# abmoRobotics/isaac_rover_orbit

Hardware: AMD Instinct MI355X
Metric: env-steps/sec AAURoverEnv-v0 @ num_envs=4096; 1/2/4/8 MI355X (higher is better)
Workload: dtype f32

## Files before the change

### isaac_rover_orbit_amd/csrc/rover_kernels.hip

```cpp
#include <hip/hip_runtime.h>
#include <vector>

#include <cmath>
#include <cstdio>
#include <cstring>
#include <new>
#include <type_traits>

#include <dlfcn.h>

#include "../../include/rover_hip.h"
#include "../../include/rover_debug.h"
#include "rover_model.hpp"
#include "rover_internal.hpp"

namespace {

struct StepConsts {
    float h, inv_h, inv_m, inv_I[3];
    float steer_hkp, steer_den_inv, steer_i_over_h, steer_dv_max;
    float wheel_den_inv, wheel_h_over_i, lt_motor;
    float bogie_keep[3], b_winv[3];
    float bogie_gq[3];
};
// ... 402 lines not shown

struct ArmConsts {
    float d0[3], axd[3], ad;
};
__device__ __forceinline__ ArmConsts make_arm(const float *wb, const float *P, const float *ax)
{
    ArmConsts a;
#pragma unroll
    for (int i = 0; i < 3; ++i) a.d0[i] = wb[i] - P[i];
    cross3f(ax, a.d0, a.axd);
    a.ad = dot3f(ax, a.d0);
    return a;
}
struct SubConsts {
    float e1[3], e2[3];
};
__device__ __forceinline__ SubConsts make_sub(const float *cj, const float *P, const float *ax)
{
    const ArmConsts a = make_arm(cj, P, ax);
    SubConsts s;
#pragma unroll
    for (int i = 0; i < 3; ++i) { s.e1[i] = fmaf(ax[i], a.ad, -a.d0[i]); s.e2[i] = a.axd[i]; }
    return s;
}
__device__ __forceinline__ float bogie_gravity(const SubConsts &sub, const float R[3][3], float sb, float cb, float gq, float bd)
{
    float vb[3];
#pragma unroll
    for (int i = 0; i < 3; ++i) vb[i] = fmaf(sub.e1[i], sb, sub.e2[i] * cb);
    const float vwz = fmaf(R[2][2], vb[2], fmaf(R[2][1], vb[1], R[2][0] * vb[0]));
    return fmaf(gq, vwz, bd);
}
__device__ __forceinline__ void bogie_sincos(float bq, float *sb, float *cb)
{
    rv_sincosf_small(bq, sb, cb);
    const bool wide = !(fabsf(bq) < 0.75f);
    if (__builtin_expect(__builtin_amdgcn_ballot_w64(wide) != 0ull, 0)) {
        float s2, c2;
        rv_sincosf(bq, &s2, &c2);
        if (wide) { *sb = s2; *cb = c2; }
    }
}
struct RowQ {
    float ja[3], jb, m;
};
__device__ __forceinline__ RowQ row_quantities(const StepConsts &k, const float R[3][3], const float *r, const float *axrp,
                                               const float *dir, bool friction_row, bool at_hi, bool at_lo, float b_winv)
{
    RowQ o;
    float x[3];
    cross3f(r, dir, x);
    mat_tvecf(R, x, o.ja);
    float jb = dot3f(dir, axrp);
    const bool lock = friction_row ? (at_hi || at_lo) : ((at_hi && jb > 0.0f) || (at_lo && jb < 0.0f));
    if (lock) jb = 0.0f;
    o.jb = jb;
    o.m = 1.0f / (RV_SPLIT_C * k.inv_m + RV_SPLIT_C * wdot3(o.ja, k.inv_I) + RV_SPLIT_B * (jb * jb * b_winv));
    return o;
}
__device__ __forceinline__ float row_coupling(const StepConsts &k, const RowQ &a, const RowQ &b, float b_winv)
{
    return RV_SPLIT_C * wdot3x(a.ja, b.ja, k.inv_I) + RV_SPLIT_B * (a.jb * b.jb * b_winv);
}
__device__ __forceinline__ float dpp_ror8(float x);
struct LinkSample {
    float h00, h01, h10, h11, o00, o01, o10, o11, fx, fy, z;
};
__device__ __forceinline__ LinkSample link_point_fetch(const RvParams &p, const float R[3][3], const float *pos, const float *P,
                                                       const float *ax, float bq, const float *p0, const float *bogie_sc = nullptr)
{
    float sb, cb;
    if (bogie_sc) { sb = bogie_sc[0]; cb = bogie_sc[1]; }
    else bogie_sincos(bq, &sb, &cb);
    const float d0[3] = {p0[0] - P[0], p0[1] - P[1], p0[2] - P[2]};
    float axd[3], pt_b[3], tmp[3];
    cross3f(ax, d0, axd);
    const float ad = dot3f(ax, d0);
#pragma unroll
    for (int i = 0; i < 3; ++i) pt_b[i] = P[i] + fmaf(ax[i], ad * (1.0f - cb), fmaf(axd[i], sb, d0[i] * cb));
    mat_vecf(R, pt_b, tmp);
    float u = ((pos[0] + tmp[0]) - p.min_x) * p.inv_res;
    float v = ((pos[1] + tmp[1]) - p.min_y) * p.inv_res;
    u = clamp_med3(u, 0.0f, (float)(p.W - 1));
    v = clamp_med3(v, 0.0f, (float)(p.H - 1));
    int j0 = (int)u, i0 = (int)v;
    if (j0 > p.W - 2) j0 = p.W - 2;
    if (i0 > p.H - 2) i0 = p.H - 2;
    const size_t base = (size_t)i0 * p.W + j0;
    const float *q = p.height + base, *o = p.obstacle + base;
    LinkSample s;
    s.fx = u - (float)j0; s.fy = v - (float)i0; s.z = pos[2] + tmp[2];
    s.h00 = q[0]; s.h01 = q[1]; s.h10 = q[p.W]; s.h11 = q[p.W + 1];
    s.o00 = o[0]; s.o01 = o[1]; s.o10 = o[p.W]; s.o11 = o[p.W + 1];
    return s;
}
__device__ __forceinline__ void link_point_eval(const LinkSample &s, float inv_res, float *force)
{
    const float dx0 = s.h01 - s.h00, dx1 = s.h11 - s.h10, dy0 = s.h10 - s.h00, dy1 = s.h11 - s.h01;
    const float hx0 = s.h00 + s.fx * dx0, hx1 = s.h10 + s.fx * dx1;
    const float hgt = hx0 + s.fy * (hx1 - hx0);
    const float gx = (dx0 + s.fy * (dx1 - dx0)) * inv_res;
    const float gy = (dy0 + s.fx * (dy1 - dy0)) * inv_res;
    const float o0 = s.o00 + s.fx * (s.o01 - s.o00), o1 = s.o10 + s.fx * (s.o11 - s.o10);
    const float obst = o0 + s.fy * (o1 - o0);
    const float pen = hgt - s.z;
    const float fk = (obst > RV_OBSTACLE_EPS && pen > 0.0f) ? RV_LINK_STIFFNESS * pen : 0.0f;
    const float fz = fk * rv_rsqrtf(fmaf(gx, gx, fmaf(gy, gy, 1.0f)));
    force[0] = -gx * fz;
    force[1] = -gy * fz;
    force[2] = fz;
}
__device__ __forceinline__ float link_sample_obstacle(const LinkSample &s)
{
    const float o0 = s.o00 + s.fx * (s.o01 - s.o00), o1 = s.o10 + s.fx * (s.o11 - s.o10);
    return o0 + s.fy * (o1 - o0);
}
__device__ __forceinline__ void link_point_force(const RvParams &p, const float R[3][3], const float *pos, const float *P,
                                                 const float *ax, float bq, const float *p0, float *force)
{
    link_point_eval(link_point_fetch(p, R, pos, P, ax, bq, p0), p.inv_res, force);
}
__device__ __forceinline__ void link_body_forces(const float lf[6][2], float *Fb )
{
    Fb[0] = (lf[0][1] + lf[1][0]) + lf[1][1];
    Fb[1] = (lf[2][1] + lf[3][0]) + lf[3][1];
    Fb[2] = lf[4][1] + lf[5][1];
    Fb[3] = lf[0][0]; Fb[4] = lf[2][0]; Fb[5] = lf[4][0]; Fb[6] = lf[5][0];
}
template <bool WANT_OBST, bool GROUP_ROLE = false>
__device__ __forceinline__ void wheel_geometry(const RvParams &p, const StepConsts &k, const float R[3][3], const float *pos,
                                               const float *com_w, const ArmConsts &arm, const float *P, const float *ax,
                                               float b_winv, float bq, bool at_hi, bool at_lo, bool steerable, float steer_q,
                                               Contact &ct, bool role_b = false, const float *bogie_sc = nullptr)
{
    const float *d0 = arm.d0, *axd = arm.axd;
    const float ad = arm.ad;
    float sb, cb;
    if (bogie_sc) { sb = bogie_sc[0]; cb = bogie_sc[1]; }
    else bogie_sincos(bq, &sb, &cb);
    float cen_b[3], cen_w[3], piv_w[3], ax_w[3], tmp[3];
#pragma unroll
    for (int i = 0; i < 3; ++i) cen_b[i] = P[i] + fmaf(ax[i], ad * (1.0f - cb), fmaf(axd[i], sb, d0[i] * cb));
    mat_vecf(R, cen_b, tmp);
#pragma unroll
    for (int i = 0; i < 3; ++i) cen_w[i] = pos[i] + tmp[i];
    mat_vecf(R, P, tmp);
#pragma unroll
    for (int i = 0; i < 3; ++i) piv_w[i] = pos[i] + tmp[i];
    mat_vecf(R, ax, ax_w);
    float hgt, gx, gy;
    ct.obst = 0.0f;
    terrain_sample<WANT_OBST>(p, cen_w[0], cen_w[1], hgt, gx, gy, ct.obst);
    const float inv = rv_rsqrtf(fmaf(gx, gx, fmaf(gy, gy, 1.0f)));
    ct.n[0] = -gx * inv; ct.n[1] = -gy * inv; ct.n[2] = inv;
    const float gap = fmaf(cen_w[2] - hgt, ct.n[2], -RV_WHEEL_CONTACT_RADIUS);
    float cp[3];
#pragma unroll
    for (int i = 0; i < 3; ++i) cp[i] = fmaf(-RV_WHEEL_CONTACT_RADIUS, ct.n[i], cen_w[i]);
    float fwd_b[3] = {1.0f, 0.0f, 0.0f}, fwd[3];
    if (steerable) rv_sincosf(steer_q, &fwd_b[1], &fwd_b[0]);
    mat_vecf(R, fwd_b, fwd);
    const float fn = dot3f(fwd, ct.n);
#pragma unroll
    for (int i = 0; i < 3; ++i) ct.t[i] = fmaf(-fn, ct.n[i], fwd[i]);
    const float tl = dot3f(ct.t, ct.t);
    const float tinv = rv_rsqrtf(fmaxf(tl, 1.0e-12f));
#pragma unroll
    for (int i = 0; i < 3; ++i) ct.t[i] *= tinv;
    cross3f(ct.n, ct.t, ct.s);
    float r[3], rp[3], x[3];
#pragma unroll
    for (int i = 0; i < 3; ++i) { r[i] = cp[i] - com_w[i]; rp[i] = cp[i] - piv_w[i]; }
    cross3f(ax_w, rp, x);
    {
        const float sep = -gap * k.inv_h;
        const float push = RV_BAUMGARTE * (-gap) * k.inv_h;
        ct.bias = gap > 0.0f ? sep : fminf(push, RV_MAX_DEPENETRATION_VEL);
    }
    if (!GROUP_ROLE) {
        const RowQ qn = row_quantities(k, R, r, x, ct.n, false, at_hi, at_lo, b_winv);
        const RowQ qt = row_quantities(k, R, r, x, ct.t, true, at_hi, at_lo, b_winv);
        const RowQ qs = row_quantities(k, R, r, x, ct.s, true, at_hi, at_lo, b_winv);
#pragma unroll
        for (int i = 0; i < 3; ++i) { ct.jn_a[i] = qn.ja[i]; ct.jt_a[i] = qt.ja[i]; ct.js_a[i] = qs.ja[i]; }
        ct.jn_b = qn.jb; ct.jt_b = qt.jb; ct.js_b = qs.jb;
        ct.mn = qn.m; ct.mt = qt.m; ct.ms = qs.m;
        ct.a_nt = row_coupling(k, qn, qt, b_winv);
        ct.a_ns = row_coupling(k, qn, qs, b_winv);
        ct.a_ts = row_coupling(k, qt, qs, b_winv);
    } else {
        const float dx[3] = {role_b ? ct.t[0] : ct.n[0], role_b ? ct.t[1] : ct.n[1], role_b ? ct.t[2] : ct.n[2]};
        const RowQ qx = row_quantities(k, R, r, x, dx, role_b, at_hi, at_lo, b_winv);
        const RowQ qs = row_quantities(k, R, r, x, ct.s, true, at_hi, at_lo, b_winv);
        const float a_xs = row_coupling(k, qx, qs, b_winv);
        RowQ qy;
#pragma unroll
        for (int i = 0; i < 3; ++i) qy.ja[i] = dpp_ror8(qx.ja[i]);
        qy.jb = dpp_ror8(qx.jb);
        qy.m = dpp_ror8(qx.m);
        const float a_ys = dpp_ror8(a_xs);
#pragma unroll
        for (int i = 0; i < 3; ++i) { ct.jn_a[i] = role_b ? qy.ja[i] : qx.ja[i]; ct.jt_a[i] = role_b ? qx.ja[i] : qy.ja[i]; ct.js_a[i] = qs.ja[i]; }
        ct.jn_b = role_b ? qy.jb : qx.jb; ct.jt_b = role_b ? qx.jb : qy.jb; ct.js_b = qs.jb;
        ct.mn = role_b ? qy.m : qx.m; ct.mt = role_b ? qx.m : qy.m; ct.ms = qs.m;
        ct.a_nt = row_coupling(k, qx, qy, b_winv);
        ct.a_ns = role_b ? a_ys : a_xs;
        ct.a_ts = role_b ? a_xs : a_ys;
    }
}

typedef float f2 __attribute__((ext_vector_type(2)));
__device__ __forceinline__ f2 fma2(f2 a, f2 b, f2 c) { return __builtin_elementwise_fma(a, b, c); }
struct RoleRows {
    f2 Jn[2];
    f2 Jts[4];
    f2 Cn, Cts;
    f2 Mn[2], Mt[2], Ms[2];
};
__device__ __forceinline__ void role_partials(const RoleRows &r, const f2 *V, float &pn, float &pt, float &ps)
{
    const f2 p = fma2(r.Jn[1], V[1], fma2(r.Jn[0], V[0], r.Cn));
    pn = p.x + p.y;
    f2 ts = fma2(r.Jts[0], (f2){V[0].x, V[0].x}, r.Cts);
    ts = fma2(r.Jts[1], (f2){V[0].y, V[0].y}, ts);
    ts = fma2(r.Jts[2], (f2){V[1].x, V[1].x}, ts);
    ts = fma2(r.Jts[3], (f2){V[1].y, V[1].y}, ts);
    pt = ts.x;
    ps = ts.y;
}
__device__ __forceinline__ void role_outputs(const RoleRows &r, float dn, float dt, float ds, f2 *o)
// ... 368 lines not shown
    "v_add_f32_dpp v252, v252, v252 row_half_mirror" RV_DPP_FULL                                                       \
    "v_add_f32_dpp v253, v253, v253 row_half_mirror" RV_DPP_FULL                                                       \
    "v_add_f32_dpp v254, v254, v254 row_half_mirror" RV_DPP_LANES_A                                                    \
    "v_add_f32_dpp v255, v255, v255 row_half_mirror" RV_DPP_LANES_A                                                    \
    "v_pk_add_f32 %[v0], %[v0], v[252:253]\n\t"                                                                      \
    "v_pk_add_f32 %[v1], %[v1], v[254:255]\n\t"

#define RV_SOLVER_ASM(TRIPS, BODY)                                                                                                \
    asm volatile(                                                                                                                 \
        ".p2align 5\n\t"                                                                                                        \
        "1:\n\t" BODY "s_cbranch_scc1 1b\n\t"                                                                                  \
        : [v0] "+v"(v0), [v1] "+v"(v1), [ln] "+v"(ln), [lt] "+v"(lt), [ls] "+v"(ls), [cnt] "+s"(TRIPS)                            \
        : [jn0] "v"(rr.Jn[0]), [jn1] "v"(rr.Jn[1]), [jts0] "v"(rr.Jts[0]), [jts1] "v"(rr.Jts[1]), [jts2] "v"(rr.Jts[2]),          \
          [jts3] "v"(rr.Jts[3]), [cn] "v"(rr.Cn), [cts] "v"(rr.Cts), [mn0] "v"(rr.Mn[0]), [mn1] "v"(rr.Mn[1]), [mt0] "v"(rr.Mt[0]), \
          [mt1] "v"(rr.Mt[1]), [ms0] "v"(rr.Ms[0]), [ms1] "v"(rr.Ms[1]), [mn] "v"(ct.mn), [mt] "v"(ct.mt), [ms] "v"(ct.ms),        \
          [ant] "v"(ct.a_nt), [ans] "v"(ct.a_ns), [ats] "v"(ct.a_ts), [mu] "s"(mu), [ltm] "s"(K.lt_motor)                         \
        : "v238", "v239", "v240", "v241", "v242", "v243", "v244", "v245", "v246", "v247", "v248", "v249", "v250", "v251",         \
          "v252", "v253", "v254", "v255", "scc")
#define RV_HALF_A(FILLER) RV_SOLVER_HALF("%[ln]", "v249", "%[lt]", "v251", "%[ls]", "v238", FILLER)
#define RV_HALF_B(FILLER) RV_SOLVER_HALF("v249", "%[ln]", "v251", "%[lt]", "v238", "%[ls]", FILLER)
#ifndef RV_SOLVER_UNROLL
#define RV_SOLVER_UNROLL 8
#endif
__device__ __forceinline__ void solver_iterations_group(const StepConsts &K, Contact &ct, const RoleRows &rr, f2 *V, float mu,
                                                        int iterations)
{
    f2 v0 = V[0], v1 = V[1];
    float ln = ct.ln, lt = ct.lt, ls = ct.ls;
    int rest = iterations;
    if (RV_SOLVER_UNROLL == 8) {
        int octs = rest >> 3;
        rest &= 7;
        if (octs > 0)
            RV_SOLVER_ASM(octs, RV_HALF_A("s_sub_u32 %[cnt], %[cnt], 1\n\t") RV_HALF_B("s_nop 0\n\t") RV_HALF_A("s_nop 0\n\t") RV_HALF_B("s_nop 0\n\t")
                                    RV_HALF_A("s_nop 0\n\t") RV_HALF_B("s_nop 0\n\t") RV_HALF_A("s_nop 0\n\t") RV_HALF_B("s_cmp_lg_u32 %[cnt], 0\n\t"));
    }
    if (RV_SOLVER_UNROLL >= 4) {
        int quads = rest >> 2;
        rest &= 3;
        if (quads > 0)
            RV_SOLVER_ASM(quads, RV_HALF_A("s_sub_u32 %[cnt], %[cnt], 1\n\t") RV_HALF_B("s_nop 0\n\t") RV_HALF_A("s_nop 0\n\t")
                                     RV_HALF_B("s_cmp_lg_u32 %[cnt], 0\n\t"));
    }
    int pairs = rest >> 1;
    if (pairs > 0) RV_SOLVER_ASM(pairs, RV_HALF_A("s_sub_u32 %[cnt], %[cnt], 1\n\t") RV_HALF_B("s_cmp_lg_u32 %[cnt], 0\n\t"));
    V[0] = v0;
    V[1] = v1;
    ct.ln = ln;
    ct.lt = lt;
    ct.ls = ls;
    if (iterations & 1) solver_iteration_generic(K, ct, rr, V, mu);
}

template <bool RECORD_FORCE, bool LINK_ELSEWHERE = false>
__device__ __forceinline__ void physics_substep_group(const RvParams &p, const StepConsts &K, GroupLane &g,
                                                      float *Fw ,
                                                      int sidx = 0)
{
    K1_STAMP(2 + 3 * sidx);
    constexpr float COM_B[3] = RV_COM_B_INIT;
    const float h = K.h;
    const float mu = p.cfg.friction_mu;
    if (g.steerable) steer_joint(K, g.steer_t, g.sq, g.sqd);
    float R[3][3], com_w[3];
#pragma unroll
    for (int i = 0; i < 3; ++i) {
        com_w[i] = g.pos[i] + g.com_off[i];
#pragma unroll
        for (int j = 0; j < 3; ++j) R[i][j] = g.R[i][j];
    }
    float v[3] = {g.linvel[0], g.linvel[1], fmaf(-RV_GRAVITY, h, g.linvel[2])};
    float w[3];
    mat_tvecf(R, g.angvel, w);
    const float bq = g.bq;
    float bd = g.bqd * g.bogie_keep;
    float bsc[2];
    bogie_sincos(bq, &bsc[0], &bsc[1]);
    bd = bogie_gravity(g.sub, R, bsc[0], bsc[1], g.bogie_gq, bd);
    const bool at_hi = bq >= RV_BOGIE_QLIM - 1.0e-5f, at_lo = bq <= -RV_BOGIE_QLIM + 1.0e-5f;
    Contact ct;
    LinkSample ls;
    if (RECORD_FORCE && !LINK_ELSEWHERE) ls = link_point_fetch(p, R, g.pos, g.P, g.ax, bq, g.lp, bsc);
    wheel_geometry<RECORD_FORCE && !LINK_ELSEWHERE, true>(p, K, R, g.pos, com_w, g.arm, g.P, g.ax, g.b_winv, bq, at_hi, at_lo, g.steerable, g.sq, ct, g.role_b, bsc);
    if (RECORD_FORCE && !LINK_ELSEWHERE) link_point_eval(ls, p.inv_res, Fw + 3);
    K1_STAMP(3 + 3 * sidx);
    ct.ln = RV_WARM_START * g.lam;
    ct.lt = 0.0f;
    ct.ls = 0.0f;
    const bool rb = g.role_b;
    RoleRows rr;
    {
        const float cw = RV_WHEEL_CONTACT_RADIUS * g.wqd;
        make_role(ct, rb, g.minv0, g.minv1, cw, rr);
    }
    f2 V[2];
    V[0] = rb ? (f2){v[2], w[2]} : (f2){v[0], w[0]};
    V[1] = rb ? (f2){bd, 0.0f} : (f2){v[1], w[1]};
    {
        const f2 l2 = {ct.ln, ct.ln};
        const f2 o0 = rr.Mn[0] * l2, o1 = rr.Mn[1] * l2;
        float a0 = o0.x, a1 = o0.y, a2 = o1.x, a3 = o1.y;
        slot_sum4(a0, a1, a2, a3);
        V[0] += (f2){a0, a1};
        V[1] += (f2){a2, a3};
    }
    solver_iterations_group(K, ct, rr, V, mu, p.cfg.solver_iterations);
    {
        const float p0x = dpp_ror8(V[0].x), p0y = dpp_ror8(V[0].y), p1x = dpp_ror8(V[1].x), p1y = dpp_ror8(V[1].y);
        v[0] = rb ? p0x : V[0].x; w[0] = rb ? p0y : V[0].y;
        v[1] = rb ? p1x : V[1].x; w[1] = rb ? p1y : V[1].y;
        v[2] = rb ? V[0].x : p0x; w[2] = rb ? V[0].y : p0y;
        bd = rb ? V[1].x : p1x;
    }
    K1_STAMP(4 + 3 * sidx);
    wheel_motor(K, g.wheel_t, ct.lt, g.wq, g.wqd);
    g.lam = ct.ln;
    if (RECORD_FORCE) {
        const bool on = LINK_ELSEWHERE ? true : ct.obst > RV_OBSTACLE_EPS;
#pragma unroll
        for (int i = 0; i < 3; ++i) Fw[i] = on ? fmaf(ct.s[i], ct.ls, fmaf(ct.t[i], ct.lt, ct.n[i] * ct.ln)) * K.inv_h : 0.0f;
    }
    chassis_integrate(h, R, v, w, com_w, g.pos, g.quat, g.linvel, g.angvel, g.R, g.com_off);
    bogie_integrate(h, bq, bd, g.bq, g.bqd);
}

struct ResetDraws {
    int32_t spawn_row;
    float yaw_u;
    const float *theta_u;
    float heading_u;
};

__device__ __forceinline__ void sample_target(const RvParams &p, float ox, float oy, uint32_t gid, uint32_t count, const float *inj_theta,
                                              float &tx_out, float &ty_out, float &tz_out)
{
    const rover_config &c = p.cfg;
// ... 778 lines not shown

template <bool TRI>
__device__ __forceinline__ void scan_single_tile_wave(const RvParams &p, int16_t *tile, int lane, int n_env, int e_base,
                                                      const PrivateWindows &w, float *__restrict__ out, int row_stride, int col0,
                                                      const float2 *__restrict__ ray_xy)
{
    if (n_env <= 0) return;
    private_issue(p, w, 0, tile, lane);
    f2 oxy[PRIVATE_ROUNDS];
#pragma unroll
    for (int m = 0; m < PRIVATE_ROUNDS; ++m) {
        const float2 v = ray_xy[m * 64 + lane];
        oxy[m] = (f2){v.x, v.y};
    }
#pragma unroll
    for (int j = 0; j < 4; ++j) {
        if (j < n_env) {
            asm volatile("s_waitcnt vmcnt(0)" ::: "memory");
            __builtin_amdgcn_wave_barrier();
            private_cast<TRI>(p, w, j, tile, lane, e_base, out, row_stride, col0, oxy, ray_xy);
            if (j + 1 < n_env) {
                asm volatile("s_waitcnt lgkmcnt(0)" ::: "memory");
                private_issue(p, w, j + 1, tile, lane);
            }
        }
    }
}

__device__ __forceinline__ void windows_to_lds(float *win, const ScanWindow &sw, int lane)
{
    if ((lane & 15) == 0) {
        float4 *d = reinterpret_cast<float4 *>(win + (lane >> 4) * 8);
        d[0] = make_float4(sw.px, sw.py, sw.pz, sw.cy);
        d[1] = make_float4(sw.sy, __int_as_float(sw.i_lo), __int_as_float(sw.j_lo), __int_as_float(sw.th | (sw.interior << 15) | (sw.tw4 << 16)));
    }
}
__device__ __forceinline__ void windows_from_lds(const float *win, PrivateWindows &w)
{
#pragma unroll
    for (int j = 0; j < 4; ++j) {
        const float4 d0 = reinterpret_cast<const float4 *>(win + j * 8)[0], d1 = reinterpret_cast<const float4 *>(win + j * 8)[1];
        auto uni = [](float v) { return __int_as_float(__builtin_amdgcn_readfirstlane(__float_as_int(v))); };
        w.px[j] = uni(d0.x); w.py[j] = uni(d0.y); w.pz[j] = uni(d0.z); w.cy[j] = uni(d0.w); w.sy[j] = uni(d1.x);
        w.i_lo[j] = __builtin_amdgcn_readfirstlane(__float_as_int(d1.y)); w.j_lo[j] = __builtin_amdgcn_readfirstlane(__float_as_int(d1.z));
        w.pk[j] = __builtin_amdgcn_readfirstlane(__float_as_int(d1.w));
    }
}
constexpr int RV_HAND = 448;
__device__ __forceinline__ float *fused_win(float *lds, const RvParams &p, int wv)
{
    return reinterpret_cast<float *>(reinterpret_cast<int16_t *>(lds) + (size_t)8 * p.tile_dim * p.tile_pitch) + wv * 64;
}
__device__ __forceinline__ float *fused_link(float *lds, const RvParams &p, int wv) { return fused_win(lds, p, 0) + 256 + wv * RV_HAND; }
template <bool TRI>
__device__ __forceinline__ void scan_copy_wave(const RvParams &p, const float *__restrict__ state, float *lds, int partner, int lane,
                                               float *__restrict__ obs, const float2 *__restrict__ ray_xy)
{
    const int tile_cells = p.tile_dim * p.tile_pitch;
    int16_t *tile0 = reinterpret_cast<int16_t *>(lds) + (size_t)(2 * partner) * tile_cells, *tile1 = tile0 + tile_cells;
    const float *win = fused_win(lds, p, partner);
    const int e_base = (int)(blockIdx.x * 4 + partner) * 4;
    const int n_env = max(0, min(4, p.n - e_base));
    PrivateWindows w;
    f2 oxy[PRIVATE_ROUNDS];
#pragma unroll
    for (int m = 0; m < PRIVATE_ROUNDS; ++m) {
        const float2 v = ray_xy[m * 64 + lane];
        oxy[m] = (f2){v.x, v.y};
    }
    {
        const int e = min(e_base + (lane >> 4), p.n - 1);
        const uint32_t count = __float_as_uint(state[(size_t)ROVER_RESET_COUNT * p.n + e]);
        ResetOutcome ro;
        reset_draw(p, (uint32_t)(p.env_id_offset + e), count, nullptr, ro);
        if ((lane & 15) == 0) {
            float4 *d = reinterpret_cast<float4 *>(fused_link(lds, p, partner) + 256 + (lane >> 4) * 12);
            d[0] = make_float4(ro.px, ro.py, ro.pz, ro.qw);
            d[1] = make_float4(ro.qz, ro.tx, ro.ty, ro.tz);
            d[2] = make_float4(ro.heading_cmd, 0.0f, 0.0f, 0.0f);
        }
    }
    {
        __syncthreads();
        const float *lk = fused_link(lds, p, partner);
        const SlotConst sc = d_SLOT[lane & 7];
        const bool role_b = (lane & 8) != 0;
        const float *pe = lk + (lane >> 4) * 12;
        const float R[3][3] = {{pe[0], pe[1], pe[2]}, {pe[3], pe[4], pe[5]}, {pe[6], pe[7], pe[8]}};
        const float pos[3] = {pe[9], pe[10], pe[11]};
        const float P[3] = {sc.P[0], sc.P[1], sc.P[2]}, ax[3] = {sc.ax[0], sc.ax[1], sc.ax[2]};
        float lp[3];
#pragma unroll
        for (int i = 0; i < 3; ++i) lp[i] = role_b ? sc.lp[1][i] : sc.lp[0][i];
        const float bq = lk[64 + lane];
        float bsc[2];
        bogie_sincos(bq, &bsc[0], &bsc[1]);
        const LinkSample ls = link_point_fetch(p, R, pos, P, ax, bq, lp, bsc);
        const float wbp[3] = {sc.wb[0], sc.wb[1], sc.wb[2]};
        const LinkSample ws = link_point_fetch(p, R, pos, P, ax, bq, wbp, bsc);
        float f3[3];
        link_point_eval(ls, p.inv_res, f3);
        const_cast<float *>(lk)[320 + lane] = f3[0];
        const_cast<float *>(lk)[384 + lane] = f3[1];
        const_cast<float *>(lk)[128 + lane] = f3[2];
        const_cast<float *>(lk)[192 + lane] = link_sample_obstacle(ws);
    }
    K1_LITE(0);
    __syncthreads();
    K1_LITE(1);
    {
// ... 32 lines not shown
        if ((lane & 15) == 0)
            *(volatile __attribute__((address_space(3))) float *)(__attribute__((address_space(3))) float *)(lk + 48 + (lane >> 4) * 4 + 3) = 3.0f;
    }
    K1_LITE(3);
    asm volatile("s_waitcnt vmcnt(0)" ::: "memory");
    K1_LITE(4);
    if (n_env > 0) private_cast<TRI>(p, w, 0, tile0, lane, e_base, obs, p.obs_w, 4, oxy, ray_xy);
    K1_LITE(5);
    asm volatile("s_waitcnt lgkmcnt(0)" ::: "memory");
    K1_LITE(6);
    K1_LITE(7);
    if (n_env > 2) private_issue(p, w, 2, tile0, lane);
    K1_LITE(8);
    asm volatile("s_waitcnt vmcnt(0)" ::: "memory");
    K1_LITE(9);
    K1_LITE(10);
    K1_LITE(11);
    if (n_env > 2) private_cast<TRI>(p, w, 2, tile0, lane, e_base, obs, p.obs_w, 4, oxy, ray_xy);
    K1_LITE(12);
    K1_LITE(13);
    K1_LITE(14);
    K1_LITE(15);
}

enum StepForm { TWO_LAUNCH, COPY_WAVES, SINGLE_TILE };
template <StepForm FORM, bool TRI, bool BEGIN_ONLY = false>
__device__ __forceinline__ void step_group_body(const RvParams &p, float *__restrict__ state, const float *__restrict__ action,
                                                float *__restrict__ obs, float *__restrict__ reward, uint8_t *__restrict__ terminated,
                                                uint8_t *__restrict__ truncated, float *__restrict__ force,
                                                float *__restrict__ log_partial, float *lds, const float2 *__restrict__ ray_xy)
{
    const int lane = threadIdx.x & 63;
    const int wave = blockIdx.x * (RV_K1G_THREADS / 64) + (threadIdx.x >> 6);
    const int e_raw = wave * 4 + (lane >> 4);
    const bool active = e_raw < p.n;
    const int e = active ? e_raw : p.n - 1;
    const int N = p.n;
    const rover_config &c = p.cfg;
    const SlotConst sc = d_SLOT[lane & 7];
    const GroupIds id = group_ids(lane, sc);
    K1_STAMP(0);
    K1_LITE(0);

    const StepConsts &K = p.K;
    GroupLane g;
    group_load(state, N, e, id, sc, K, g, p.cfg.mass_model);
    float act[2], prev[2];
    prev[0] = state[(size_t)(ROVER_ACTION + 0) * N + e];
    prev[1] = state[(size_t)(ROVER_ACTION + 1) * N + e];
    const float2 a = reinterpret_cast<const float2 *>(action)[e];
    act[0] = a.x;
    act[1] = a.y;
    float S[ROVER_STATE_WORDS];
    {
        float processed[2], steer[4], rim[6];
        ackermann_core(c, act, processed, steer, rim);
        const float steer_m[4] = {steer[0], steer[3], steer[1], steer[2]};
        const float rim_m[6] = {rim[1], rim[5], rim[0], rim[4], rim[2], rim[3]};
        float st = steer_m[0], rv = rim_m[0];
#pragma unroll
        for (int i = 1; i < 4; ++i) st = (id.si == i) ? steer_m[i] : st;
#pragma unroll
        for (int i = 1; i < 6; ++i) rv = (id.k == i) ? rim_m[i] : rv;
        g.steer_t = st;
        g.wheel_t = rv / c.wheel_radius;
    }
    float Fw[6] = {0.0f, 0.0f, 0.0f, 0.0f, 0.0f, 0.0f};
    f2 oxy[PRIVATE_ROUNDS];
    K1_STAMP(1);
    for (int s = 0; s < c.decimation - 1; ++s) physics_substep_group<false>(p, K, g, nullptr, s);
#pragma unroll
    for (int i = ROVER_TARGET_W; i < ROVER_ACTION; ++i) S[i] = state[(size_t)i * N + e];
#pragma unroll
    for (int i = ROVER_TIME_LEFT; i < ROVER_LAMBDA_N; ++i) S[i] = state[(size_t)i * N + e];
    S[ROVER_RESET_COUNT] = state[(size_t)ROVER_RESET_COUNT * N + e];
    if constexpr (FORM == COPY_WAVES) {
        const int wv = __builtin_amdgcn_readfirstlane((int)(threadIdx.x >> 6));
        float *lk = fused_link(lds, p, wv);
        if ((lane & 15) == 0) {
            float4 *d = reinterpret_cast<float4 *>(lk + (lane >> 4) * 12);
            d[0] = make_float4(g.R[0][0], g.R[0][1], g.R[0][2], g.R[1][0]);
            d[1] = make_float4(g.R[1][1], g.R[1][2], g.R[2][0], g.R[2][1]);
            d[2] = make_float4(g.R[2][2], g.pos[0], g.pos[1], g.pos[2]);
        }
        lk[64 + lane] = g.bq;
        __syncthreads();
        if (c.decimation > 0) physics_substep_group<true, true>(p, K, g, Fw, c.decimation - 1);
    } else {
        if (c.decimation > 0) physics_substep_group<true>(p, K, g, Fw, c.decimation - 1);
    }
    K1_STAMP(20);
    K1_LITE(1);
    if constexpr (FORM == COPY_WAVES) {
        const int wv = __builtin_amdgcn_readfirstlane((int)(threadIdx.x >> 6));
        float *lk = fused_link(lds, p, wv);
        if ((lane & 15) == 0) {
            float4 *d = reinterpret_cast<float4 *>(lk + 48 + (lane >> 4) * 4);
            float4 *q = reinterpret_cast<float4 *>(lk + 304 + (lane >> 4) * 4);
            d[0] = make_float4(g.pos[0], g.pos[1], g.pos[2], 0.0f);
            q[0] = make_float4(g.quat[0], g.quat[1], g.quat[2], g.quat[3]);
        }
        __syncthreads();
        if (c.decimation > 0) {
            const int wv = __builtin_amdgcn_readfirstlane((int)(threadIdx.x >> 6));
            const float *lk = fused_link(lds, p, wv);
            Fw[3] = lk[320 + lane]; Fw[4] = lk[384 + lane]; Fw[5] = lk[128 + lane];
            if (!(lk[192 + lane] > RV_OBSTACLE_EPS)) { Fw[0] = 0.0f; Fw[1] = 0.0f; Fw[2] = 0.0f; }
        }
    }
    if (!id.wheel_active) { Fw[0] = 0.0f; Fw[1] = 0.0f; Fw[2] = 0.0f; Fw[3] = 0.0f; Fw[4] = 0.0f; Fw[5] = 0.0f; }
    float F[ROVER_NUM_BODIES * 3];
#pragma unroll
    for (int i = 0; i < ROVER_NUM_BODIES * 3; ++i) F[i] = 0.0f;
    const bool any_force = __ballot(Fw[0] != 0.0f || Fw[1] != 0.0f || Fw[2] != 0.0f || Fw[5] != 0.0f) != 0ull;
    if (__builtin_expect(any_force, 0)) {
        constexpr int BODY_SLOT[6] = {1, 3, 0, 2, 4, 5};
        const int base = lane & ~15;
#pragma unroll
        for (int b = 0; b < 6; ++b)
#pragma unroll
            for (int i = 0; i < 3; ++i) F[(7 + b) * 3 + i] = __shfl(Fw[i], base + BODY_SLOT[b], 64);
#pragma unroll
        for (int i = 0; i < 3; ++i) {
            float lf[6][2], Fb[7];
#pragma unroll
            for (int sl = 0; sl < 6; ++sl) {
                lf[sl][0] = __shfl(Fw[3 + i], base + sl, 64);
                lf[sl][1] = __shfl(Fw[3 + i], base + 8 + sl, 64);
            }
            link_body_forces(lf, Fb);
#pragma unroll
            for (int b = 0; b < 7; ++b) F[b * 3 + i] = Fb[b];
        }
    }
    int coll_known = -1;
    if constexpr (FORM == COPY_WAVES) {
        const int wv = __builtin_amdgcn_readfirstlane((int)(threadIdx.x >> 6));
        const bool coll = any_force ? collision_measure(F) > 1.0f : false;
        coll_known = coll ? 1 : 0;
        bool term_e[ROVER_NUM_TERM];
// ... 178 lines not shown
                __builtin_amdgcn_s_sleep(1);
            }
        }
        windows_from_lds(win, pw);
        K1_LITE(5);
        K1_STAMP(27);
        if (n_scan > 1) {
            private_issue(p, pw, 1, tile1, lane);
            asm volatile("s_waitcnt vmcnt(0)" ::: "memory");
            private_cast<TRI>(p, pw, 1, tile1, lane, e_base, obs, p.obs_w, 4, oxy, ray_xy);
            asm volatile("s_waitcnt lgkmcnt(0)" ::: "memory");
        }
        K1_STAMP(28);
        K1_LITE(6);
        K1_LITE(7);
        if (n_scan > 3) {
            private_issue(p, pw, 3, tile1, lane);
            K1_LITE(8);
            asm volatile("s_waitcnt vmcnt(0)" ::: "memory");
            K1_STAMP(29);
            K1_LITE(9);
            private_cast<TRI>(p, pw, 3, tile1, lane, e_base, obs, p.obs_w, 4, oxy, ray_xy);
        }
        K1_STAMP(26);
        K1_LITE(10);
    }
}
__global__ __launch_bounds__(RV_K1G_THREADS) void rover_step_begin_kernel(RvParams p, float *__restrict__ state,
                                                                          const float *__restrict__ action, float *__restrict__ reward,
                                                                          uint8_t *__restrict__ terminated, uint8_t *__restrict__ truncated,
                                                                          float *__restrict__ force)
{
    step_group_body<TWO_LAUNCH, false, true>(p, state, action, nullptr, reward, terminated, truncated, force, nullptr, nullptr, nullptr);
}
__global__ __launch_bounds__(RV_K1G_THREADS) void rover_step_kernel_group(RvParams p, float *__restrict__ state,
                                                              const float *__restrict__ action, float *__restrict__ obs,
                                                              float *__restrict__ reward, uint8_t *__restrict__ terminated,
                                                              uint8_t *__restrict__ truncated, float *__restrict__ force,
                                                              float *__restrict__ log_partial)
{
    step_group_body<TWO_LAUNCH, false>(p, state, action, obs, reward, terminated, truncated, force, log_partial, nullptr, nullptr);
}
template <bool TRI>
__global__ __launch_bounds__(2 * RV_K1G_THREADS) RV_FUSED_ATTR void rover_step_scan_kernel(
    RvParams p, float *__restrict__ state, const float *__restrict__ action, float *__restrict__ obs, float *__restrict__ reward,
    uint8_t *__restrict__ terminated, uint8_t *__restrict__ truncated, float *__restrict__ force, float *__restrict__ log_partial,
    const float2 *__restrict__ ray_xy)
{
    extern __shared__ __align__(16) float lds[];
    const int wv = __builtin_amdgcn_readfirstlane((int)(threadIdx.x >> 6));
    if (wv < RV_K1G_THREADS / 64) {
        step_group_body<COPY_WAVES, TRI>(p, state, action, obs, reward, terminated, truncated, force, log_partial, lds, ray_xy);
    } else {
        scan_copy_wave<TRI>(p, state, lds, wv - RV_K1G_THREADS / 64, (int)(threadIdx.x & 63), obs, ray_xy);
    }
}

__global__ __launch_bounds__(RV_K1G_THREADS) void rover_physics_kernel_group(RvParams p, float *__restrict__ state,
                                                                             const float *steer_t, const float *wheel_t,
                                                                             int substeps, float *force)
{
    const int lane = threadIdx.x & 63;
    const int e_raw = (blockIdx.x * (RV_K1G_THREADS / 64) + (threadIdx.x >> 6)) * 4 + (lane >> 4);
    const bool active = e_raw < p.n;
    const int e = active ? e_raw : p.n - 1;
    const int N = p.n;
    const SlotConst sc = d_SLOT[lane & 7];
    const GroupIds id = group_ids(lane, sc);
    const StepConsts &K = p.K;
    GroupLane g;
    group_load(state, N, e, id, sc, K, g, p.cfg.mass_model);
    g.steer_t = steer_t[4 * e + (id.si >= 0 ? id.si : 0)];
    g.wheel_t = wheel_t[6 * e + id.k];
    float Fw[6] = {0.0f, 0.0f, 0.0f, 0.0f, 0.0f, 0.0f};
    for (int s = 0; s < substeps - 1; ++s) physics_substep_group<false>(p, K, g, nullptr);
    if (substeps > 0) physics_substep_group<true>(p, K, g, Fw);
    if (!id.wheel_active) { Fw[3] = 0.0f; Fw[4] = 0.0f; Fw[5] = 0.0f; }
    if (active) group_store(state, N, e, id, g, lane);
    if (force && active && id.owner) {
#pragma unroll
        for (int i = 0; i < 3; ++i) force[(size_t)(id.body * 3 + i) * N + e] = Fw[i];
    }
    if (force) {
        const int base = lane & ~15;
#pragma unroll
        for (int i = 0; i < 3; ++i) {
            float lf[6][2], Fb[7];
#pragma unroll
            for (int sl = 0; sl < 6; ++sl) {
                lf[sl][0] = __shfl(Fw[3 + i], base + sl, 64);
                lf[sl][1] = __shfl(Fw[3 + i], base + 8 + sl, 64);
            }
            link_body_forces(lf, Fb);
            if (active && (lane & 15) < 7) {
                float fb = Fb[0];
#pragma unroll
                for (int b = 1; b < 7; ++b) fb = ((lane & 15) == b) ? Fb[b] : fb;
                force[(size_t)((lane & 15) * 3 + i) * N + e] = fb;
            }
        }
    }
}

__global__ __launch_bounds__(64) void rover_reset_kernel(RvParams p, float *__restrict__ state, const uint8_t *mask,
                                                         const int32_t *spawn_row, const float *yaw_u, const float *theta_u,
                                                         const float *heading_u)
{
// ... 1252 lines not shown
```

Baseline: 103.5 million.

## Offload steering joint integration and sincos to copy waves via LDS handoff

In the fused scan kernel, the copy waves now precompute the steering-joint integration and steering sin/cos for every substep. They write the results into spare LDS tile rows and publish them through an LDS flag word. The physics waves spin-wait on that flag after the first substep, then read the precomputed steering values instead of recomputing them, which takes that work off the physics critical path. It adds a __syncthreads in the copy path, a spin loop with sleep, and reuse of tile LDS that must not overlap the scan's use of it. There are also small branch-to-select rewrites in row_quantities and in the bias computation.

```diff
diff --git a/isaac_rover_orbit_amd/csrc/rover_kernels.hip b/isaac_rover_orbit_amd/csrc/rover_kernels.hip
--- a/isaac_rover_orbit_amd/csrc/rover_kernels.hip
+++ b/isaac_rover_orbit_amd/csrc/rover_kernels.hip
@@ -478,8 +478,10 @@
     cross3f(r, dir, x);
     mat_tvecf(R, x, o.ja);
     float jb = dot3f(dir, axrp);
-    const bool lock = friction_row ? (at_hi || at_lo) : ((at_hi && jb > 0.0f) || (at_lo && jb < 0.0f));
-    if (lock) jb = 0.0f;
+    const bool lock_n = (at_hi & (jb > 0.0f)) | (at_lo & (jb < 0.0f));
+    const bool lock_f = at_hi | at_lo;
+    const bool lock = friction_row ? lock_f : lock_n;
+    jb = lock ? 0.0f : jb;
     o.jb = jb;
     o.m = 1.0f / (RV_SPLIT_C * k.inv_m + RV_SPLIT_C * wdot3(o.ja, k.inv_I) + RV_SPLIT_B * (jb * jb * b_winv));
     return o;
@@ -557,7 +559,8 @@
 __device__ __forceinline__ void wheel_geometry(const RvParams &p, const StepConsts &k, const float R[3][3], const float *pos,
                                                const float *com_w, const ArmConsts &arm, const float *P, const float *ax,
                                                float b_winv, float bq, bool at_hi, bool at_lo, bool steerable, float steer_q,
-                                               Contact &ct, bool role_b = false, const float *bogie_sc = nullptr)
+                                               Contact &ct, bool role_b = false, const float *bogie_sc = nullptr,
+                                               const float *steer_sc = nullptr)
 {
     const float *d0 = arm.d0, *axd = arm.axd;
     const float ad = arm.ad;
@@ -584,7 +587,8 @@
 #pragma unroll
     for (int i = 0; i < 3; ++i) cp[i] = fmaf(-RV_WHEEL_CONTACT_RADIUS, ct.n[i], cen_w[i]);
     float fwd_b[3] = {1.0f, 0.0f, 0.0f}, fwd[3];
-    if (steerable) rv_sincosf(steer_q, &fwd_b[1], &fwd_b[0]);
+    if (steer_sc) { fwd_b[1] = steer_sc[0]; fwd_b[0] = steer_sc[1]; }
+    else if (steerable) rv_sincosf(steer_q, &fwd_b[1], &fwd_b[0]);
     mat_vecf(R, fwd_b, fwd);
     const float fn = dot3f(fwd, ct.n);
 #pragma unroll
@@ -601,7 +605,8 @@
     {
         const float sep = -gap * k.inv_h;
         const float push = RV_BAUMGARTE * (-gap) * k.inv_h;
-        ct.bias = gap > 0.0f ? sep : fminf(push, RV_MAX_DEPENETRATION_VEL);
+        const float push_c = fminf(push, RV_MAX_DEPENETRATION_VEL);
+        ct.bias = gap > 0.0f ? sep : push_c;
     }
     if (!GROUP_ROLE) {
         const RowQ qn = row_quantities(k, R, r, x, ct.n, false, at_hi, at_lo, b_winv);
@@ -1076,16 +1081,31 @@
     if (iterations & 1) solver_iteration_generic(K, ct, rr, V, mu);
 }
 
-template <bool RECORD_FORCE, bool LINK_ELSEWHERE = false>
+template <bool RECORD_FORCE, bool LINK_ELSEWHERE = false, bool STEER_ELSEWHERE = false>
 __device__ __forceinline__ void physics_substep_group(const RvParams &p, const StepConsts &K, GroupLane &g,
                                                       float *Fw ,
-                                                      int sidx = 0)
+                                                      int sidx = 0, bool steer_handed = false, const float2 *steer_hand = nullptr)
 {
     K1_STAMP(2 + 3 * sidx);
     constexpr float COM_B[3] = RV_COM_B_INIT;
     const float h = K.h;
     const float mu = p.cfg.friction_mu;
-    if (g.steerable) steer_joint(K, g.steer_t, g.sq, g.sqd);
+    float ssc[2];
+    if constexpr (STEER_ELSEWHERE) {
+        if (__builtin_expect(steer_handed, 1)) {
+            const float2 sc2 = steer_hand[0];
+            ssc[0] = sc2.x; ssc[1] = sc2.y;
+            if (RECORD_FORCE) {
+                const float2 fin = steer_hand[64];
+                g.sq = fin.x; g.sqd = fin.y;
+            }
+        } else {
+            ssc[0] = 0.0f; ssc[1] = 1.0f;
+            if (g.steerable) { steer_joint(K, g.steer_t, g.sq, g.sqd); rv_sincosf(g.sq, &ssc[0], &ssc[1]); }
+        }
+    } else {
+        if (g.steerable) steer_joint(K, g.steer_t, g.sq, g.sqd);
+    }
     float R[3][3], com_w[3];
 #pragma unroll
     for (int i = 0; i < 3; ++i) {
@@ -1105,7 +1125,8 @@
     Contact ct;
     LinkSample ls;
     if (RECORD_FORCE && !LINK_ELSEWHERE) ls = link_point_fetch(p, R, g.pos, g.P, g.ax, bq, g.lp, bsc);
-    wheel_geometry<RECORD_FORCE && !LINK_ELSEWHERE, true>(p, K, R, g.pos, com_w, g.arm, g.P, g.ax, g.b_winv, bq, at_hi, at_lo, g.steerable, g.sq, ct, g.role_b, bsc);
+    wheel_geometry<RECORD_FORCE && !LINK_ELSEWHERE, true>(p, K, R, g.pos, com_w, g.arm, g.P, g.ax, g.b_winv, bq, at_hi, at_lo, g.steerable, g.sq, ct, g.role_b, bsc,
+                                                          STEER_ELSEWHERE ? ssc : nullptr);
     if (RECORD_FORCE && !LINK_ELSEWHERE) link_point_eval(ls, p.inv_res, Fw + 3);
     K1_STAMP(3 + 3 * sidx);
     ct.ln = RV_WARM_START * g.lam;
@@ -1990,10 +2011,68 @@
     return reinterpret_cast<float *>(reinterpret_cast<int16_t *>(lds) + (size_t)8 * p.tile_dim * p.tile_pitch) + wv * 64;
 }
 __device__ __forceinline__ float *fused_link(float *lds, const RvParams &p, int wv) { return fused_win(lds, p, 0) + 256 + wv * RV_HAND; }
+__device__ __forceinline__ void lane_targets(const rover_config &c, const float *act, int si, int k, float &steer_t, float &wheel_t)
+{
+    float processed[2], steer[4], rim[6];
+    ackermann_core(c, act, processed, steer, rim);
+    const float steer_m[4] = {steer[0], steer[3], steer[1], steer[2]};
+    const float rim_m[6] = {rim[1], rim[5], rim[0], rim[4], rim[2], rim[3]};
+    float st = steer_m[0], rv = rim_m[0];
+#pragma unroll
+    for (int i = 1; i < 4; ++i) st = (si == i) ? steer_m[i] : st;
+#pragma unroll
+    for (int i = 1; i < 6; ++i) rv = (k == i) ? rim_m[i] : rv;
+    steer_t = st;
+    wheel_t = rv / c.wheel_radius;
+}
+
+__device__ __forceinline__ bool steer_hand_on(const RvParams &p)
+{
+    return p.cfg.decimation >= 2 && (size_t)p.cfg.decimation * 64 * sizeof(float2) <= (size_t)p.tile_dim * p.tile_pitch * sizeof(int16_t);
+}
+__device__ __forceinline__ float2 *steer_hand_rows(float *lds, const RvParams &p, int wv)
+{
+    return reinterpret_cast<float2 *>(reinterpret_cast<int16_t *>(lds) + (size_t)(2 * wv + 1) * p.tile_dim * p.tile_pitch);
+}
+typedef volatile __attribute__((address_space(3))) float *lds_word_ptr;
+__device__ __forceinline__ lds_word_ptr steer_hand_word(float *lds, const RvParams &p, int wv)
+{
+    return (lds_word_ptr)(__attribute__((address_space(3))) float *)(fused_win(lds, p, wv) + 32);
+}
+__device__ __forceinline__ void copy_wave_steering(const RvParams &p, const float *__restrict__ state, const float *__restrict__ action,
+                                                   float *lds, int partner, int lane)
+{
+    const rover_config &c = p.cfg;
+    const int N = p.n;
+    const int e = min((int)(blockIdx.x * 4 + partner) * 4 + (lane >> 4), N - 1);
+    const SlotConst sc = d_SLOT[lane & 7];
+    const bool steerable = sc.si >= 0;
+    const int si = steerable ? sc.si : 0;
+    float q = state[(size_t)(ROVER_STEER_Q + si) * N + e], qd = state[(size_t)(ROVER_STEER_QD + si) * N + e];
+    const float2 a = reinterpret_cast<const float2 *>(action)[e];
+    const float act[2] = {a.x, a.y};
+    float steer_t, wheel_t;
+    lane_targets(c, act, sc.si, sc.k, steer_t, wheel_t);
+    float2 *row = steer_hand_rows(lds, p, partner) + lane;
+    for (int s = 0; s < c.decimation; ++s) {
+        if (steerable) steer_joint(p.K, steer_t, q, qd);
+        if (s > 0) {
+            float sn = 0.0f, cs = 1.0f;
+            if (steerable) rv_sincosf(q, &sn, &cs);
+            row[(s - 1) * 64] = make_float2(sn, cs);
+        }
+    }
+    row[(c.decimation - 1) * 64] = make_float2(q, qd);
+    __builtin_amdgcn_fence(__ATOMIC_RELEASE, "workgroup");
+    if (lane == 0) *steer_hand_word(lds, p, partner) = 1.0f;
+}
 template <bool TRI>
-__device__ __forceinline__ void scan_copy_wave(const RvParams &p, const float *__restrict__ state, float *lds, int partner, int lane,
-                                               float *__restrict__ obs, const float2 *__restrict__ ray_xy)
-{
+__device__ __forceinline__ void scan_copy_wave(const RvParams &p, const float *__restrict__ state, const float *__restrict__ action,
+                                               float *lds, int partner, int lane, float *__restrict__ obs,
+                                               const float2 *__restrict__ ray_xy)
+{
+    __syncthreads();
+    if (steer_hand_on(p)) copy_wave_steering(p, state, action, lds, partner, lane);
     const int tile_cells = p.tile_dim * p.tile_pitch;
     int16_t *tile0 = reinterpret_cast<int16_t *>(lds) + (size_t)(2 * partner) * tile_cells, *tile1 = tile0 + tile_cells;
     const float *win = fused_win(lds, p, partner);
@@ -2132,23 +2211,34 @@
     act[0] = a.x;
     act[1] = a.y;
     float S[ROVER_STATE_WORDS];
-    {
-        float processed[2], steer[4], rim[6];
-        ackermann_core(c, act, processed, steer, rim);
-        const float steer_m[4] = {steer[0], steer[3], steer[1], steer[2]};
-        const float rim_m[6] = {rim[1], rim[5], rim[0], rim[4], rim[2], rim[3]};
-        float st = steer_m[0], rv = rim_m[0];
-#pragma unroll
-        for (int i = 1; i < 4; ++i) st = (id.si == i) ? steer_m[i] : st;
-#pragma unroll
-        for (int i = 1; i < 6; ++i) rv = (id.k == i) ? rim_m[i] : rv;
-        g.steer_t = st;
-        g.wheel_t = rv / c.wheel_radius;
-    }
+    lane_targets(c, act, id.si, id.k, g.steer_t, g.wheel_t);
     float Fw[6] = {0.0f, 0.0f, 0.0f, 0.0f, 0.0f, 0.0f};
     f2 oxy[PRIVATE_ROUNDS];
     K1_STAMP(1);
-    for (int s = 0; s < c.decimation - 1; ++s) physics_substep_group<false>(p, K, g, nullptr, s);
+    bool steer_hand = false;
+    const float2 *steer_rows = nullptr;
+    if constexpr (FORM == COPY_WAVES) {
+        const int wv = __builtin_amdgcn_readfirstlane((int)(threadIdx.x >> 6));
+        if (lane == 0) *steer_hand_word(lds, p, wv) = 0.0f;
+        __syncthreads();
+        steer_hand = steer_hand_on(p);
+        steer_rows = steer_hand_rows(lds, p, wv) + lane;
+        for (int s = 0; s < c.decimation - 1; ++s) {
+            physics_substep_group<false, false, true>(p, K, g, nullptr, s, steer_hand && s > 0, steer_rows + (s - 1) * 64);
+            if (steer_hand && s == 0) {
+                const lds_word_ptr word = steer_hand_word(lds, p, wv);
+#pragma unroll 1
+                for (int spin = 0; spin < (1 << 20); ++spin) {
+                    if (__builtin_amdgcn_ballot_w64(*word != 1.0f) == 0ull) break;
+                    __builtin_amdgcn_s_sleep(1);
+                }
+                __builtin_amdgcn_fence(__ATOMIC_ACQUIRE, "workgroup");
+            }
+        }
+        steer_rows += (c.decimation - 2) * 64;
+    } else {
+        for (int s = 0; s < c.decimation - 1; ++s) physics_substep_group<false>(p, K, g, nullptr, s);
+    }
 #pragma unroll
     for (int i = ROVER_TARGET_W; i < ROVER_ACTION; ++i) S[i] = state[(size_t)i * N + e];
 #pragma unroll
@@ -2165,7 +2255,7 @@
         }
         lk[64 + lane] = g.bq;
         __syncthreads();
-        if (c.decimation > 0) physics_substep_group<true, true>(p, K, g, Fw, c.decimation - 1);
+        if (c.decimation > 0) physics_substep_group<true, true, true>(p, K, g, Fw, c.decimation - 1, steer_hand, steer_rows);
     } else {
         if (c.decimation > 0) physics_substep_group<true>(p, K, g, Fw, c.decimation - 1);
     }
@@ -2450,7 +2540,7 @@
     if (wv < RV_K1G_THREADS / 64) {
         step_group_body<COPY_WAVES, TRI>(p, state, action, obs, reward, terminated, truncated, force, log_partial, lds, ray_xy);
     } else {
-        scan_copy_wave<TRI>(p, state, lds, wv - RV_K1G_THREADS / 64, (int)(threadIdx.x & 63), obs, ray_xy);
+        scan_copy_wave<TRI>(p, state, action, lds, wv - RV_K1G_THREADS / 64, (int)(threadIdx.x & 63), obs, ray_xy);
     }
 }
 
```

Result: no change. 102.9 million (-0.5%).
